# y9c/cutseq

Hardware: AMD Instinct MI355X
Metric: M read-pairs/sec (higher is better)
Workload: dtype u8

## Files before the change

### cutseq_amd/csrc/cutseq_hip.hip

```cpp
#include <hip/hip_runtime.h>

#include <cmath>
#include <cstdarg>
#include <cstdio>
#include <cstdlib>
#include <cstring>
#include <algorithm>
#include <atomic>
#include <map>
#include <new>
#include <string>
#include <thread>
#include <vector>

#include <sys/mman.h>

#include "../../include/cutseq_hip.h"
#include "trim_kernel.hip.inc"
#include "long_kernel.hip.inc"
#include "text_kernels.hip.inc"
#include "deflate_kernels.hip.inc"
#include "info_kernels.hip.inc"

namespace {
// ... 450 lines not shown
  for (int m = 0; m < 2; ++m)
    for (int i = 0; i < cnt[m]; ++i) {
      int rc = build_dev_op(src[m][i], p->host.ops[m][i], i, m + 1);
      if (rc) {
        delete p;
        return rc;
      }
    }
  for (int m = 0; m < 2; ++m) {
    bool seen = false;
    for (int i = 0; i < cnt[m]; ++i) {
      if (seen) p->host.ops[m][i].exists_only = 0;
      seen = seen || p->host.ops[m][i].exists_only != 0;
    }
  }
  bool coded = true;
  for (int m = 0; m < 2; ++m)
    for (int i = 0; i < cnt[m]; ++i) {
      const cs_op &op = p->host.ops[m][i].op;
      if (op.kind != CS_OP_ADAPTER) continue;
      for (int j = 0; j < op.m; ++j) coded = coded && is_acgt(op.seq[j]);
    }
  p->host.coded = coded ? 1 : 0;
  if (coded)
    for (int m = 0; m < 2; ++m)
      for (int i = 0; i < cnt[m]; ++i) {
        csdev::DevOp &d = p->host.ops[m][i];
        if (d.op.kind != CS_OP_ADAPTER) continue;
        for (int j = 0; j < d.op.m; ++j) d.op.seq[j] = (uint8_t)csdev::base_code(d.op.seq[j]);
        d.base_char = csdev::base_code(d.base_char);
      }
  static_assert(csdev::kFnibDwords == 6, "DevOp::fnib");
  for (int m = 0; m < 2; ++m)
    for (int i = 0; i < cnt[m]; ++i) {
      csdev::DevOp &d = p->host.ops[m][i];
      memset(d.eq_tab, 0, sizeof d.eq_tab);
      memset(d.fnib, 0, sizeof d.fnib);
      if (d.op.kind != CS_OP_ADAPTER) continue;
      const int mm = d.op.m;
      for (int ent = 0; ent < 4; ++ent) {
        const int which = (ent == 0) ? 0 : (ent == 1) ? 1 : (ent == 2) ? 3 : 2;
        const uint64_t mask = d.peq[which];
        d.eq_tab[ent * 2] = (uint32_t)mask;
        d.eq_tab[ent * 2 + 1] = (mm >= 1 && mm <= 32) ? ((uint32_t)mask << (32 - mm)) : (uint32_t)(mask >> 32);
      }
      if (coded)
        for (int idx = 0; idx < mm && idx < 32; ++idx)
          d.fnib[idx >> 3] |= (uint32_t)((d.op.seq[d.op.reversed ? mm - 1 - idx : idx] >> 3) & 7u) << (4 * (idx & 7));
    }
  for (int m = 0; m < 2; ++m)
    for (int i = 0; i < cnt[m]; ++i) {
      csdev::DevOp &d = p->host.ops[m][i];
      if (d.op.kind != CS_OP_CUT) continue;
      auto pack = [](const cs_op &o) {
        return (uint32_t)(uint16_t)o.cut_len | ((uint32_t)(o.conditional ? 1u : 0u) << 16) | ((uint32_t)(o.capture & 3u) << 17) |
               ((uint32_t)(o.force_min_len > 0x1fff ? 0x1fffu : o.force_min_len) << 19);
      };
      d.cut_run = 1;
      d.cut_pack[0] = pack(d.op);
    }
  {
    const char *env = getenv("CUTSEQ_CUT_RUNS");
    if (!(env && atoi(env) == 0))
      for (int m = 0; m < 2; ++m)
        for (int i = 0; i < cnt[m];) {
          if (p->host.ops[m][i].op.kind != CS_OP_CUT) {
            ++i;
            continue;
          }
          int j = i;
          while (j < cnt[m] && j - i < csdev::kCutRun && p->host.ops[m][j].op.kind == CS_OP_CUT) {
            p->host.ops[m][i].cut_pack[j - i] = p->host.ops[m][j].cut_pack[0];
            ++j;
          }
          p->host.ops[m][i].cut_run = (uint32_t)(j - i);
          i = j;
        }
  }
  {
    const char *env = getenv("CUTSEQ_PAIR");
    const bool allow = coded && !(env && atoi(env) == 0);
    const char *env_log = getenv("CUTSEQ_LOG_ALWAYS");
    const bool log_always = env_log && atoi(env_log) != 0;
    auto log_friendly = [log_always](int mm, int kk) {
      if (log_always) return true;
      double variants = 0, choose = 1, pw = 1;
      for (int e = 0; e <= kk && e <= mm; ++e) {
        variants += choose * pw;
        choose = choose * (double)(mm - e) / (double)(e + 1);
        pw *= 6.0;
      }
      double space = 1;
      for (int i = 0; i < mm; ++i) space *= 4.0;
      return 300.0 * variants / space < 0.03;
    };
    for (int m = 0; m < 2; ++m) {
      if (allow && cnt[m] >= 1) {
        csdev::DevOp &f = p->host.ops[m][0];
        const bool free_ends = (f.op.align_flags & (CS_QUERY_START | CS_QUERY_STOP)) == (CS_QUERY_START | CS_QUERY_STOP);
        if (f.op.kind == CS_OP_ADAPTER && f.filter_mode == csdev::FILTER_MYERS32 && !f.op.reversed && free_ends &&
            f.op.shortcut == CS_SHORTCUT_NONE && !f.exists_only && log_friendly(f.op.m, f.op.k)) {
          f.solo_first = 1;
          f.quiet_groups = (uint32_t)csdev::quiet_columns((int)f.op.align_flags, f.op.m, f.op.k, nullptr) / 8u;
        }
      }
      if (!allow || cnt[m] < 2) continue;
      csdev::DevOp &a = p->host.ops[m][0];
      const csdev::DevOp &b = p->host.ops[m][1];
      const int ma = a.op.m, ka = a.op.k, mo = a.op.min_overlap;
      const bool ends_free = (b.op.align_flags & (CS_QUERY_START | CS_QUERY_STOP)) == (CS_QUERY_START | CS_QUERY_STOP);
      if (!a.exists_only || a.op.kind != CS_OP_ADAPTER || b.op.kind != CS_OP_ADAPTER || b.exists_only ||
          b.filter_mode != csdev::FILTER_MYERS32 || b.op.reversed || !ends_free || b.op.shortcut != CS_SHORTCUT_NONE ||
          ma + ka > 31 || ka > 14 || !log_friendly(b.op.m, b.op.k))
        continue;
      a.pair_next = 1;
      for (int ent = 0; ent < 4; ++ent) {
        const int which = (ent == 0) ? 0 : (ent == 1) ? 1 : (ent == 2) ? 3 : 2;
        uint32_t fwd = 0;
        for (int i = 0; i < ma; ++i)
          if ((a.peq[which] >> (ma - 1 - i)) & 1ull) fwd |= 1u << i;
        a.eq_fwd[ent] = fwd << (32 - ma);
      }
      for (int j = 1; j <= 32; ++j) {
        int best = -1;
        if (j > ma + ka) best = ka;
        else
          for (int i = mo; i <= ma; ++i) {
            const int d = i > j ? i - j : j - i;
            if (d <= (int)a.op.thr[i] && (int)a.op.thr[i] > best) best = a.op.thr[i];
          }
        a.pair_tn[(j - 1) >> 3] |= (uint32_t)(best + 1) << (4 * ((j - 1) & 7));
      }
      a.quiet_groups = (uint32_t)csdev::quiet_columns((int)b.op.align_flags, b.op.m, b.op.k, a.pair_tn) / 8u;
    }
  }
  *out = p;
  return CS_OK;
}

void cs_plan_destroy(cs_plan *plan) { delete plan; }

int cs_plan_set_max_n(cs_plan *plan, double count) {
  if (!plan) return fail(CS_ERR_ARG, "null plan");
  if (!(count >= 0.0)) return fail(CS_ERR_ARG, "max_n %g: the count must not be negative or NaN", count);
  plan->host.max_n_on = 1;
  plan->host.max_n = count;
  return CS_OK;
}

int cs_plan_set_max_length(cs_plan *plan, uint32_t length) {
  if (!plan) return fail(CS_ERR_ARG, "null plan");
  plan->host.max_length_on = 1;
  plan->host.max_length = length;
  return CS_OK;
}

int cs_plan_set_max_ee(cs_plan *plan, double errors) {
  if (!plan) return fail(CS_ERR_ARG, "null plan");
  if (!(errors >= 0.0)) return fail(CS_ERR_ARG, "max_ee %g: the bound must not be negative or NaN", errors);
  plan->host.max_ee_on = 1;
  plan->host.max_ee = errors;
  for (int b = 0; b < 256; ++b) plan->host.ee_table[b] = pow(10.0, (double)(33 - b) / 10.0);
  return CS_OK;
}

int cs_plan_set_ee_reversed(cs_plan *plan, int reversed) {
  if (!plan) return fail(CS_ERR_ARG, "null plan");
  plan->host.ee_reversed = reversed ? 1u : 0u;
  return CS_OK;
}

int cs_plan_walk_info(const cs_plan *plan, int mate, uint32_t info[6]) {
  if (!plan || !info) return fail(CS_ERR_ARG, "null plan or info");
  if (mate < 1 || mate > 2) return fail(CS_ERR_ARG, "mate %d: 1 or 2", mate);
  memset(info, 0, 6 * sizeof info[0]);
  if (plan->host.n_ops[mate - 1] < 1) return CS_OK;
  const csdev::DevOp &a = plan->host.ops[mate - 1][0];
  info[0] = a.pair_next ? 2u : a.solo_first ? 1u : 0u;
  info[1] = a.quiet_groups;
  for (int i = 0; i < 4; ++i) info[2 + i] = a.pair_tn[i];
  return CS_OK;
}

int cs_plan_set_demux(cs_plan *plan, int mate, int op_index, const uint16_t *table, size_t entries) {
  if (!plan || !table) return fail(CS_ERR_ARG, "null plan or table");
  if (mate < 1 || mate > 2 || op_index < 0 || op_index >= plan->host.n_ops[mate - 1])
    return fail(CS_ERR_ARG, "mate %d op %d: no such op", mate, op_index);
  const cs_op &op = plan->host.ops[mate - 1][op_index].op;
  if (op.kind != CS_OP_DEMUX) return fail(CS_ERR_ARG, "mate %d op %d is not a CS_OP_DEMUX op", mate, op_index);
  if (plan->host.ops[mate - 1][op_index].filter_mode)
    return fail(CS_ERR_ARG, "mate %d op %d: m + k = %d > %d (or CS_DEMUX_BY_OPS) takes cs_plan_set_demux_ops, not a table", mate,
                op_index, op.m + op.k, CS_DEMUX_MAX_PREFIX);
  size_t want = 0, pw = 1;
  for (int l = 0; l <= op.m + op.k; ++l, pw *= 5) want += pw;
  if (entries != want) return fail(CS_ERR_ARG, "demux table: %zu entries, expected %zu for m + k = %d", entries, want, op.m + op.k);
  try {
    plan->demux[mate - 1][op_index].assign(table, table + entries);
  } catch (const std::bad_alloc &) {
    return fail(CS_ERR_NOMEM, "out of memory");
  }
  return CS_OK;
}

namespace {

struct DemuxSegment {
  std::vector<uint8_t> pool;
  std::vector<std::pair<size_t, uint32_t>> first;
};

struct DemuxWalk {
  const std::vector<std::string> &digits;
  int m, k, depth;
  const std::vector<size_t> &block;

  struct Alive {
// ... 1488 lines not shown
```

### cutseq_amd/csrc/trim_kernel.hip.inc

```

#include <type_traits>

namespace csdev {

#ifdef CS_PHASE_TIMERS
struct PhaseTimer {
  uint64_t last;
  uint32_t acc[8];
  uint32_t passes, steps, items;
};
#define CS_T_MARK(T, PHASE)                                   \
  {                                                           \
    const uint64_t cs_now = clock64();                        \
    (T).acc[PHASE] += (uint32_t)(cs_now - (T).last);          \
    (T).last = cs_now;                                        \
  }
#else
#define CS_T_MARK(T, PHASE)
#endif


constexpr int kWave = 64;

constexpr uint32_t kScoreBias = 1024u, kOriginBias = 4096u;
constexpr uint32_t kCostShift = 24, kScoreShift = 13;
constexpr uint32_t kCellZero = (kScoreBias << kScoreShift) | kOriginBias;
constexpr uint32_t kDeltaMatch = 1u << kScoreShift;
constexpr uint32_t kDeltaMismatch = (1u << kCostShift) - (1u << kScoreShift);
constexpr uint32_t kDeltaIndel = (1u << kCostShift) - (2u << kScoreShift);

enum { FILTER_NONE = 0, FILTER_MYERS32 = 1, FILTER_MYERS64 = 2, FILTER_POLY_TAIL = 3, FILTER_POLY_HEAD = 4 };

__host__ __device__ constexpr uint32_t base_code(uint32_t ascii) {
  const uint32_t sel = (ascii >> 1) & 3u;
  const bool ok = ascii == 'A' || ascii == 'C' || ascii == 'G' || ascii == 'T';
  return (sel << 3) | (ok ? 0u : 32u);
}
constexpr int kEqTableBytes = 64;
constexpr int kWaveItemDwords = 4;
constexpr int kCutRun = 4;
constexpr int kQCutoffLow = -1, kQCutoffHigh = 256, kQTermMax = 256;

struct DevFields {
  uint32_t kind, align_flags, reversed, remove, shortcut, match_flag, required, conditional, capture, homopolymer,
      q_base, stat_slot, m, k, min_overlap, force_min_len;
  int32_t cut_len, q_cutoff;
  int32_t length;
};

struct DevOp {
  cs_op op;
  DevFields f;
  uint64_t peq[4];
  uint32_t filter_mode;
  uint32_t base_char;
  uint32_t acgt_only;
  uint32_t thr_mul;
  uint64_t thr_step[2];
  uint32_t eq_tab[kEqTableBytes / 4];
  uint32_t fnib[6];
  uint32_t exists_only;
  uint32_t pair_next;
  uint32_t solo_first;
  uint32_t pair_tn[4];
  uint32_t eq_fwd[4];
  uint32_t cut_run;
  uint32_t cut_pack[kCutRun];
  uint32_t quiet_groups;
};

__host__ __device__ inline int quiet_columns(int flags, int m, int k, const uint32_t *tn) {
  if (flags & CS_REF_START) return 0;
  int q = 0;
  while (q + 8 < m - k && q + 8 <= 32) {
    bool clear = true;
    for (int j = q > 0 ? q : 1; j < q + 8 && tn; ++j)
      clear = clear && ((tn[(j - 1) >> 3] >> (4 * ((j - 1) & 7))) & 15u) == 0u;
    if (!clear) break;
    q += 8;
  }
  return q;
}

struct DevPlan {
  cs_params params;
  int32_t n_ops[2];
  int32_t coded;
  int32_t max_n_on;
  DevOp ops[2][CS_MAX_OPS];
  double max_n;
  uint32_t max_length_on, max_length;
  uint32_t max_ee_on, ee_reversed;
  double max_ee;
  double ee_table[256];
};

constexpr int kMaxPlanSlots = 8;
__constant__ DevPlan c_plans[kMaxPlanSlots];

struct MateArgs {
  const uint32_t *seq;
  const uint8_t *qual;
  const uint16_t *len;
  cs_result *out;
  cs_cap2 *cap2;
  uint8_t *bc;
  uint8_t *xflags;
};

constexpr uint32_t kTileCounters = 8, kTileCounterStride = 32;

struct KArgs {
  MateArgs mate[2];
  unsigned long long *stats;
  uint32_t n_reads;
  uint32_t stride_dw;
  uint32_t lds_stride_dw;
  uint32_t col_dwords;
  uint32_t plan_slot;
  uint32_t *tile_counter;
  uint32_t n_table_ops;
  uint32_t big_tiles;
  uint32_t big_shift, small_shift;
  uint32_t static_units;
  uint4 *defer[2];
  uint32_t batch_knob;
  uint32_t *defer_count;
  uint32_t defer_cap;
  const unsigned long long *gate;
  uint32_t item_slots;
  uint32_t fast_recode;
};

__device__ __forceinline__ uint32_t cell_pack(int cost, int score, int origin) {
  return ((uint32_t)cost << kCostShift) | ((uint32_t)(score + (int)kScoreBias) << kScoreShift) |
         (uint32_t)(origin + (int)kOriginBias);
}
__device__ __forceinline__ int cell_cost(uint32_t c) { return (int)(c >> kCostShift); }
__device__ __forceinline__ int cell_score(uint32_t c) { return (int)((c >> kScoreShift) & 0x7ffu) - (int)kScoreBias; }
__device__ __forceinline__ int cell_origin(uint32_t c) { return (int)(c & 0x1fffu) - (int)kOriginBias; }
constexpr uint32_t kStripScoreBias = 256u, kStripPrioShift = 22;
constexpr uint32_t kStripZero = (kStripScoreBias << kScoreShift) | kOriginBias;
__device__ __forceinline__ uint32_t strip_pack(int cost, int score, int origin) {
  return ((uint32_t)cost << kCostShift) | ((uint32_t)(score + (int)kStripScoreBias) << kScoreShift) |
         (uint32_t)(origin + (int)kOriginBias);
}
__device__ __forceinline__ int strip_score(uint32_t c) {
  return (int)((c >> kScoreShift) & 0x1ffu) - (int)kStripScoreBias;
}

__device__ __forceinline__ int thr_of(const DevOp &d, int L) {
// ... 746 lines not shown
      }
    };
    {
      const uint32_t word = take();
#pragma unroll
      for (int u = 0; u < NB; ++u) q[u] = lookup(word_code<true>(word, DIR > 0 ? u : NB - 1 - u));
      advance();
    }
    __builtin_amdgcn_s_setprio(PRIO_LOOP);
    do {
      const uint32_t word = take();
      advance();
#pragma unroll
      for (int u = 0; u < NB; ++u) {
        myers_step_noscore<false>(st, q[u], 0u);
        q[u] = lookup(word_code<true>(word, DIR > 0 ? u : NB - 1 - u));
        if (u == 3 || u == 7) sample(4);
      }
      j += NB;
    } while (j + NB - 1 <= n);
    __builtin_amdgcn_s_setprio(PRIO_REST);
    int since = 0;
#pragma unroll
    for (int u = 0; u < NB - 1; ++u) {
      if (j <= n) {
        myers_step_noscore<false>(st, q[u], 0u);
        ++j;
        ++since;
        if (since == 4) {
          sample(4);
          since = 0;
        }
      }
    }
    if (since) sample(since);
  } else {
    for (; j <= n; ++j) {
      myers_step_noscore<false>(st, lookup(row_code<true>(row, pos)), 0u);
      pos += DIR;
    }
    if (n > 0) sample(n);
  }
  CS_T_MARK(pt, 1);
  bool none = lowest > 2 * k;
  if (n > 0) {
    const int first_i = RE ? 0 : m;
    const int lo_i = max(first_i, min_overlap);
    const uint32_t pv0 = st.Pv >> sh, mv0 = st.Mv >> sh;
    const int skip = min(max(lo_i - 1, 0), m);
    int cost = 0, thr_i = 0;
    uint32_t pv = pv0, mv = mv0;
    if (skip > 0) {
      const uint32_t below = (skip >= 32) ? ~0u : ((1u << skip) - 1u);
      cost += __popc(pv & below) - __popc(mv & below);
      pv = (skip >= 32) ? 0u : (pv >> skip);
      mv = (skip >= 32) ? 0u : (mv >> skip);
      thr_i = thr_of(d, skip);
    }
    bool any = false;
    for (int i = skip + 1; i <= m; ++i) {
      cost += (int)(pv & 1u) - (int)(mv & 1u);
      pv >>= 1;
      mv >>= 1;
      thr_i += thr_step_bit(d, i);
      any = any || cost <= thr_i;
    }
    none = none && !any;
  }
  return none;
}

__device__ __forceinline__ unsigned long long lds_read_u64(uint32_t addr) { return *(const lds_u64 *)(uintptr_t)addr; }
typedef __attribute__((address_space(3))) uint8_t lds_u8;
__device__ __forceinline__ void lds_write_u8(uint32_t addr, uint32_t imm, uint32_t value) {
  *(lds_u8 *)(uintptr_t)(addr + imm) = (uint8_t)value;
}
__device__ __forceinline__ uint32_t lds_read_u8(uint32_t addr) { return *(const lds_u8 *)(uintptr_t)addr; }
__device__ __forceinline__ uint32_t pk_min_u16(uint32_t a, uint32_t b) {
  uint32_t r;
  asm("v_pk_min_u16 %0, %1, %2" : "=v"(r) : "v"(a), "v"(b));
  return r;
}

struct ItemLog {
  uint32_t slot0;
  uint32_t bytes;
  uint32_t tag_off;
};

template <bool HAS_A>
__device__ __forceinline__ Verdict myers_pair(const DevOp &da, const DevOp &db, int rule, const uint32_t *fnib_b,
                                               const uint32_t *row, int e, bool &a_none, const ItemLog &il CS_T_PARAM) {
  constexpr int NB = 8;
  constexpr int s = 0;
  const int n = e - s;
  const int m = db.f.m, k = db.f.k;
  const bool RS = db.f.align_flags & CS_REF_START;
  const int sh = 32 - m;
  MyersState<uint32_t> st;
  st.Mv = 0;
  st.Pv = RS ? 0u : (m >= 32 ? ~0u : ((1u << m) - 1u));
  const int k1 = k + 1;
  st.score = (RS ? 0 : m) - k1;
  st.Pv = (st.Pv << sh) | ((1u << sh) - 1u);
  const bool exact_by_score = !RS;
  int jfirst = -1, jlast = -1;
  int cmin = 0x7fff, jmin = -1;
  bool tie_next = false;
  uint32_t slot = il.slot0;
  const uint32_t slot_end = il.slot0 + il.bytes;
  bool log_full = false;
  const int ma = da.f.m, ka = da.f.k;
  const int sha = 32 - ma, free_a = ma - (int)da.f.min_overlap;
  MyersState<uint32_t> sa;
  sa.Mv = 0;
  sa.Pv = (((ma >= 32 ? ~0u : ((1u << ma) - 1u)) & ~((1u << free_a) - 1u)) << sha) | ((1u << sha) - 1u);
  sa.score = ma - free_a;
  int flag = 0;
  const uint32_t tn0 = da.pair_tn[0], tn1 = da.pair_tn[1], tn2 = da.pair_tn[2], tn3 = da.pair_tn[3];
  const uint32_t fill_a = (uint32_t)sha, cst4 = (uint32_t)(4 + 2 * ka + 1);
  auto sample_a = [&](uint32_t cst) {
    const int cur = (int)__builtin_popcount(sa.Pv) - (int)(__builtin_popcount(sa.Mv) + fill_a);
    flag |= sa.score + cur - (int)cst;
    sa.score = cur;
  };
  const unsigned long long tn_lo = ((unsigned long long)tn1 << 32) | tn0, tn_hi = ((unsigned long long)tn3 << 32) | tn2;
  auto tn_of = [tn_lo, tn_hi, ka](int j) -> int {
    int t1 = ka + 1;
    if (__ballot(j <= 32)) {
      const unsigned long long w = j <= 16 ? tn_lo : tn_hi;
      const int tj = (int)((uint32_t)(w >> (((uint32_t)(j - 1) & 15u) * 4u)) & 15u);
      t1 = j > 32 ? t1 : tj;
    }
    return t1;
  };
  auto column = [&](uint32_t eb, uint32_t ea, int j) {
    myers_step_la<false>(st, eb, 0u);
    if constexpr (HAS_A) {
      myers_step_la<false>(sa, ea, 0u);
      flag |= sa.score - tn_of(j);
    }
    if (st.score < 0) {
      if (jfirst < 0) jfirst = j;
      jlast = j;
      if (j == jmin + 1 && st.score + k1 == cmin) tie_next = true;
      if (st.score + k1 < cmin) {
        cmin = st.score + k1;
        jmin = j;
        tie_next = false;
      }
    }
  };
  int j = 1;
  if (n >= NB) {
    int wi = 0;
    auto take = [&]() -> uint32_t { return row[wi]; };
    auto advance = [&]() { wi += 1; };
#ifndef CS_PAIR_DEPTH
#define CS_PAIR_DEPTH 2
#endif
    constexpr int QD = CS_PAIR_DEPTH;
    static_assert(NB % QD == 0, "a group's columns must map onto the slots the same way in every group");
    uint32_t qb[QD], qa[QD];
    auto refill = [&](int slot, uint32_t code) {
      const unsigned long long pr = lds_read_u64(code);
      qb[slot] = (uint32_t)pr;
      qa[slot] = (uint32_t)(pr >> 32);
    };
    uint32_t wcur = take();
    advance();
#pragma unroll
    for (int u = 0; u < QD; ++u) refill(u, word_code<true>(wcur, u));
    constexpr int STEADY = 0, EARLY_G = 1, QUIET = 2;
    auto group = [&](auto body_tag, uint32_t tw) {
      constexpr bool EARLY = decltype(body_tag)::value == EARLY_G;
      const uint32_t wnext = take();
      advance();
      if constexpr (decltype(body_tag)::value == QUIET) {
#pragma unroll
        for (int u = 0; u < NB; ++u) {
          myers_step_noscore<false>(st, qb[u % QD], 0u);
          if constexpr (HAS_A) myers_step_noscore<false>(sa, qa[u % QD], 0u);
          refill(u % QD, u + QD < NB ? word_code<true>(wcur, u + QD) : word_code<true>(wnext, u + QD - NB));
        }
        wcur = wnext;
        j += NB;
        return;
      }
      int sc[NB];
#pragma unroll
      for (int u = 0; u < NB; ++u) {
        myers_step_la<false>(st, qb[u % QD], 0u);
        sc[u] = st.score;
        if constexpr (HAS_A && EARLY) {
          myers_step_la<false>(sa, qa[u % QD], 0u);
          flag |= sa.score - (int)((tw >> (4 * u)) & 15u);
        } else if constexpr (HAS_A) {
          myers_step_noscore<false>(sa, qa[u % QD], 0u);
          if (u == 3 || u == 7) sample_a(cst4);
        }
        refill(u % QD, u + QD < NB ? word_code<true>(wcur, u + QD) : word_code<true>(wnext, u + QD - NB));
      }
      wcur = wnext;
      constexpr uint32_t kOr3 = 0xFEu;
      uint32_t any = __builtin_amdgcn_bitop3_b32((uint32_t)sc[0], (uint32_t)sc[1], (uint32_t)sc[2], kOr3);
      any = __builtin_amdgcn_bitop3_b32(any, (uint32_t)sc[3], (uint32_t)sc[4], kOr3);
      any = __builtin_amdgcn_bitop3_b32(any, (uint32_t)sc[5], (uint32_t)sc[6], kOr3);
      any |= (uint32_t)sc[7];
      if ((int)any < 0) {
        if (slot < slot_end) {
#pragma unroll
          for (int u = 0; u < NB; ++u) lds_write_u8(slot, (uint32_t)u, (uint32_t)sc[u]);
          lds_write_u8((slot >> 3) + il.tag_off, 0u, (uint32_t)(j >> 3));
        }
        slot += 8u;
      }
      j += NB;
    };
    __builtin_amdgcn_s_setprio(PRIO_LOOP);
    const int early_groups = (ma + ka + NB - 1) >> 3;
    const int quiet_j = (int)da.quiet_groups * NB + 1;
    if (quiet_j > 1) {
      do group(std::integral_constant<int, QUIET>{}, 0u);
      while (j < quiet_j && j + NB - 1 <= n);
      st.score = (int)__builtin_popcount(st.Pv) - (int)(__builtin_popcount(st.Mv) + (uint32_t)sh) - k1;
      if constexpr (HAS_A) {
        sa.score = (int)__builtin_popcount(sa.Pv) - (int)(__builtin_popcount(sa.Mv) + fill_a);
        const int tq = (int)(da.pair_tn[da.quiet_groups - 1u] >> 28);
        flag |= sa.score - (j == quiet_j ? tq : 0);
      }
    }
    if constexpr (HAS_A) {
      int g = (int)da.quiet_groups;
      while (g < early_groups && j + NB - 1 <= n) {
        group(std::integral_constant<int, EARLY_G>{}, g == 0 ? tn0 : g == 1 ? tn1 : g == 2 ? tn2 : tn3);
        ++g;
      }
    }
    while (j + NB - 1 <= n) group(std::integral_constant<int, STEADY>{}, 0u);
    __builtin_amdgcn_s_setprio(PRIO_REST);
    if (j <= n) {
      int sc[NB];
#pragma unroll
      for (int u = 0; u < NB - 1; ++u) {
        sc[u] = 0x7f;
        if (j + u <= n) {
          uint32_t eb, ea;
          if (u < QD) {
            eb = qb[u];
            ea = qa[u];
          } else {
            const unsigned long long pr = lds_read_u64(word_code<true>(wcur, u));
            eb = (uint32_t)pr;
            ea = (uint32_t)(pr >> 32);
          }
          myers_step_la<false>(st, eb, 0u);
          sc[u] = st.score;
          if constexpr (HAS_A) {
            myers_step_la<false>(sa, ea, 0u);
            flag |= sa.score - tn_of(j + u);
          }
        }
      }
      sc[NB - 1] = 0x7f;
      int any = sc[0];
#pragma unroll
      for (int u = 1; u < NB - 1; ++u) any |= sc[u];
      if (any < 0) {
        if (slot < slot_end) {
#pragma unroll
          for (int u = 0; u < NB; ++u) lds_write_u8(slot, (uint32_t)u, (uint32_t)sc[u]);
          lds_write_u8((slot >> 3) + il.tag_off, 0u, (uint32_t)(j >> 3));
        }
        slot += 8u;
      }
      j = n + 1;
    }
    {
      const uint32_t m80 = 0x80808080u, ones = 0x01010101u;
      const uint32_t stop_at = min(slot, slot_end);
      uint32_t rd = il.slot0;
      while (__ballot(rd < stop_at)) {
        if (rd < stop_at) {
          const unsigned long long sc8 = lds_read_u64(rd);
          const int jg = (int)lds_read_u8((rd >> 3) + il.tag_off) * 8 + 1;
          rd += 8u;
          const uint32_t clo = (uint32_t)sc8 & m80, chi = (uint32_t)(sc8 >> 32) & m80;
          const uint32_t plo = (uint32_t)sc8 ^ m80, phi = (uint32_t)(sc8 >> 32) ^ m80;
          const unsigned long long c64 = ((unsigned long long)chi << 32) | clo;
          if (jfirst < 0) jfirst = jg + (__builtin_ctzll(c64) >> 3);
          jlast = jg + ((63 - __builtin_clzll(c64)) >> 3);
          const uint32_t h00ff = 0x00ff00ffu;
          const uint32_t a0 = plo & h00ff, a1 = (plo >> 8) & h00ff, b0 = phi & h00ff, b1 = (phi >> 8) & h00ff;
          const uint32_t m4 = pk_min_u16(pk_min_u16(a0, a1), pk_min_u16(b0, b1));
          const uint32_t gbyte = min(m4 & 0xffffu, m4 >> 16);
          const int gmin = (int)gbyte - 128 + k1;
          if (jmin == jg - 1 && (int)(plo & 0xffu) - 128 + k1 == cmin) tie_next = true;
          if (gmin < cmin) {
            const uint32_t gb = __builtin_amdgcn_perm(0u, gbyte, 0u);
            const uint32_t xlo = plo ^ gb, xhi = phi ^ gb;
            const uint32_t zlo = (xlo - ones) & ~xlo & m80, zhi = (xhi - ones) & ~xhi & m80;
            const int pos = __builtin_ctzll(((unsigned long long)zhi << 32) | zlo) >> 3;
            cmin = gmin;
            jmin = jg + pos;
            const unsigned long long flipped = ((unsigned long long)phi << 32) | plo;
            tie_next = pos < 7 && (uint32_t)((flipped >> (8 * (pos + 1))) & 0xffull) == gbyte;
          }
        }
      }
      log_full = slot > slot_end;
    }
  } else {
    for (int pos = s; j <= n; ++j, ++pos) {
      const unsigned long long pr = lds_read_u64(row_code<true>(row, pos));
      column((uint32_t)pr, (uint32_t)(pr >> 32), j);
    }
  }
  CS_T_MARK(pt, 1);
  a_none = flag >= 0 && !log_full;
  st.score += k1;
  const int exact_end = (exact_by_score && cmin == 0) ? jmin : -1;
  return myers_verdict<uint32_t, +1, true, true>(db, rule, fnib_b, row, s, e, st, jfirst, jlast, exact_end, cmin, jmin, tie_next);
}

__device__ __forceinline__ uint32_t foreign_flags(const uint32_t *row, int di, uint32_t xrep, int lo, int hi) {
  const uint32_t x = row[di] ^ xrep;
  const uint32_t t = (x | (x >> 1) | (x >> 2)) & 0x11111111u;
  const int first = max(lo - 8 * di, 0), last = min(hi - 8 * di, 8);
  const uint32_t upto = (last >= 8) ? 0xffffffffu : ((1u << (4 * last)) - 1u);
  return t & upto & ~((1u << (4 * first)) - 1u);
}

struct PolyBest {
  bool have;
  int origin, cost, score, len, where;
};

template <bool CODED>
__device__ __forceinline__ Verdict poly_tail(const DevOp &d, int rule, const uint32_t *row, int s, int e) {
  Verdict v = verdict_none(d.f.m);
  const int n = e - s, m = d.f.m, k = d.f.k, min_overlap = d.f.min_overlap;
  const uint32_t X = d.base_char;
  const int lim = min(n, m);
  PolyBest best = {false, 0, 0, 0, 0, 0};
  auto consider = [&](int i, int cost, int score, int origin) {
    if (i >= min_overlap && cost <= thr_of(d, i) &&
        better_candidate(rule, m, best.have, best.origin, best.cost, best.score, best.len, cost, score, origin, i)) {
      best.have = true;
      best.origin = origin;
      best.cost = cost;
      best.score = score;
      best.len = i;
    }
  };
  int b = 0, i_hi = 0;
  if (!CODED) {
    for (int i = 1; i <= lim; ++i) {
      const int nb = b + ((row_code<CODED>(row, e - i) != X) ? 1 : 0);
      if (nb > k) break;
      b = nb;
      i_hi = i;
    }
  } else {
    const uint32_t xrep = (X >> 3) * 0x11111111u;
    const int lo = e - lim;
    for (int di = (e - 1) >> 3; di >= (lo >> 3); --di) {
      const uint32_t f = foreign_flags(row, di, xrep, lo, e);
      const int c = __popc(f);
      const int seg_lo = max(lo, 8 * di);
      if (b + c <= k) {
        b += c;
        i_hi = e - seg_lo;
        continue;
      }
      for (int pos = min(e, 8 * di + 8) - 1; pos >= seg_lo; --pos) {
        const int nb = b + (int)((f >> (4 * (pos - 8 * di))) & 1u);
        if (nb > k) break;
        b = nb;
        i_hi = e - pos;
      }
      break;
    }
  }
  if (i_hi == n && n < m) {
    for (int i = m; i > n; --i) {
      const int cost = (i - n) + b;
      if (cost <= k) consider(i, cost, n - 2 * b, 0);
    }
  }
  if (!CODED) {
    for (int i = i_hi; i >= 1; --i) {
      consider(i, b, i - 2 * b, n - i);
      b -= (row_code<CODED>(row, e - i) != X) ? 1 : 0;
    }
  } else if (i_hi > 0) {
    const uint32_t xrep = (X >> 3) * 0x11111111u;
    const int lo = e - i_hi;
    uint32_t carry = 0;
    for (int di = lo >> 3; di <= ((e - 1) >> 3); ++di) {
      const uint32_t f = foreign_flags(row, di, xrep, lo, e);
      const int c = __popc(f);
      const int seg_lo = max(lo, 8 * di), seg_hi = min(e, 8 * di + 8);
      const int i_left = e - seg_lo;
// ... 678 lines not shown
    if (d == d0) keep &= 0x80808080u << ((s & 3) * 8);
    if (d == d1) keep &= 0x80808080u >> ((3 - ((e - 1) & 3)) * 8);
    const uint32_t x = (row[d] & 0xdfdfdfdfu) ^ 0x4e4e4e4eu;
    n += (uint32_t)__popc(~(((x & 0x7f7f7f7fu) + 0x7f7f7f7fu) | x) & keep);
  }
  return n;
}
__device__ __forceinline__ uint32_t count_n_nibbles(const uint32_t *row, int s, int e) {
  uint32_t n = 0;
  if (e <= s) return 0;
  const int d0 = s >> 3, d1 = (e - 1) >> 3;
  for (int d = d0; d <= d1; ++d) {
    uint32_t keep = 0x11111111u;
    if (d == d0) keep &= 0x11111111u << ((s & 7) * 4);
    if (d == d1) keep &= 0x11111111u >> ((7 - ((e - 1) & 7)) * 4);
    const uint32_t w = row[d];
    n += (uint32_t)__popc(w & (w >> 1) & (w >> 2) & keep);
  }
  return n;
}
__device__ __forceinline__ bool too_many_n(uint32_t n, int len, double count) {
  if (count < 1.0) return len > 0 && (double)n / (double)len > count;
  return (double)n > count;
}
__device__ __forceinline__ double expected_errors(const uint32_t *qrow, int s, int e, const double *table, bool reversed) {
  double ee = 0.0;
  if (e <= s) return ee;
  const int d0 = s >> 2, d1 = (e - 1) >> 2;
  if (!reversed) {
    for (int d = d0; d <= d1; ++d) {
      const uint32_t w = qrow[d];
#pragma unroll
      for (int b = 0; b < 4; ++b) {
        const int p = 4 * d + b;
        if (p >= s && p < e) ee += table[(w >> (8 * b)) & 0xffu];
      }
    }
  } else {
    for (int d = d1; d >= d0; --d) {
      const uint32_t w = qrow[d];
#pragma unroll
      for (int b = 3; b >= 0; --b) {
        const int p = 4 * d + b;
        if (p >= s && p < e) ee += table[(w >> (8 * b)) & 0xffu];
      }
    }
  }
  return ee;
}

enum { MODE_SCAN = 0, MODE_RESOLVE = 1 };

#ifndef CS_SCAN_WAVES
#define CS_SCAN_WAVES 5
#endif
enum { FILT_NONE = 0, FILT_MAXN = 1, FILT_ALL = 2, FILT_ENDS = 3, FILT_NEXTSEQ = 4, FILT_SHORTEN = 5 };
template <bool CODED, bool WIDE, int MODE, int FILT>
__global__ void __launch_bounds__(64, MODE == MODE_RESOLVE ? 4 : CS_SCAN_WAVES) trim_kernel(KArgs a) {
  if (a.gate && *a.gate != ~0ull) return;
  const DevPlan *plan = &c_plans[a.plan_slot];
  extern __shared__ uint32_t smem[];
  constexpr int TILE = kWave;
  constexpr bool SCAN = MODE != MODE_RESOLVE;
  const int tid = threadIdx.x;
  const int mate = blockIdx.y;
  const MateArgs &ma = a.mate[mate];
  const int n_ops = plan->n_ops[mate];
  const uint32_t pw0 = (uint32_t)__builtin_amdgcn_readfirstlane((int)reinterpret_cast<const uint32_t *>(&plan->params)[1]);
  const uint32_t pw1 = (uint32_t)__builtin_amdgcn_readfirstlane((int)reinterpret_cast<const uint32_t *>(&plan->params)[2]);
  static_assert(offsetof(cs_params, min_length) == 4 && offsetof(cs_params, select_rule) == 6 && offsetof(cs_params, use_filter) == 7 &&
                offsetof(cs_params, case_rule) == 8 && offsetof(cs_params, indel_tie) == 9, "cs_params layout");
  const int min_length = (int)(pw0 & 0xffffu);
  const int rule = (int)((pw0 >> 16) & 0xffu);
  const bool use_filter = ((pw0 >> 24) & 0xffu) != 0;
  const bool fold_case = (pw1 & 0xffu) == CS_CASE_FOLD;
  const bool tie_ins = ((pw1 >> 8) & 0xffu) == CS_TIE_INSERTION;
#ifdef CS_PHASE_TIMERS
  const int lane = tid;
#endif

  if (lds_addr_of(smem) != 0u) __builtin_trap();
  __builtin_amdgcn_s_setprio(SCAN ? PRIO_REST : PRIO_RESOLVE);
  uint32_t *cur_tab = smem;
  uint32_t *tile = smem + 20;
  uint32_t *col = tile + (size_t)TILE * a.lds_stride_dw;
  uint32_t *wq = col + a.col_dwords;
  uint32_t *tables = wq + (SCAN ? 0 : kWave * kWaveItemDwords);
  uint32_t *fnibs = tables + a.n_table_ops * (kEqTableBytes / 4);
  uint32_t *sacc = fnibs + a.n_table_ops * kFnibDwords;
  (void)col;
  (void)wq;

  for (int i = tid; i < (int)a.n_table_ops * (kEqTableBytes / 4); i += TILE) {
    const int t = i >> 4;
    tables[i] = t < n_ops ? plan->ops[mate][t].eq_tab[i & 15] : 0u;
  }
  for (int i = tid; i < (int)a.n_table_ops * kFnibDwords; i += TILE) {
    const int t = i / kFnibDwords, w = i - t * kFnibDwords;
    fnibs[i] = (CODED && t < n_ops) ? plan->ops[mate][t].fnib[w] : 0u;
  }
  for (int i = tid; i < kStatWords; i += TILE) sacc[i] = 0;
  if (SCAN && CODED && tid < 4) smem[16 + tid] = (n_ops > 0 && plan->ops[mate][0].pair_next) ? plan->ops[mate][0].eq_fwd[tid] : 0u;

  const uint32_t n_records = SCAN ? 0u : a.defer_count[mate * kTileCounterStride];
  uint32_t batch_rows = TILE;
  if (!SCAN) {
    if (n_records < a.batch_knob * 64u * (uint32_t)gridDim.x) batch_rows = 32;
    if (n_records < a.batch_knob * 32u * (uint32_t)gridDim.x) batch_rows = 16;
  }
  const uint32_t n_refl = SCAN ? 0u : a.defer_count[(4u + (uint32_t)mate) * kTileCounterStride];
  const uint32_t tiles_a = (n_records + batch_rows - 1) / batch_rows;
  const uint32_t n_tiles = SCAN ? (a.n_reads + (uint32_t)TILE - 1) / (uint32_t)TILE : tiles_a + (n_refl + (uint32_t)TILE - 1) / (uint32_t)TILE;
  const uint32_t big_tiles = a.big_tiles, big_units = big_tiles >> a.big_shift;
  const uint32_t big_mask = (1u << a.big_shift) - 1u, small_mask = (1u << a.small_shift) - 1u;
  auto unit_start = [&](uint32_t u) -> uint32_t {
    return (u < big_units) ? (u << a.big_shift) : big_tiles + ((u - big_units) << a.small_shift);
  };
  auto unit_end = [&](uint32_t tile) -> uint32_t {
    return (tile < big_tiles) ? ((tile | big_mask) + 1u) : big_tiles + (((tile - big_tiles) | small_mask) + 1u);
  };
  uint32_t *next_slot = sacc + kStatWords;
  const uint32_t n_counters = min(kTileCounters, (uint32_t)gridDim.x);
  const uint32_t my_counter = blockIdx.x % n_counters;
  uint32_t *counter = a.tile_counter + ((uint32_t)mate * kTileCounters + my_counter) * kTileCounterStride;
  uint32_t *claim = a.defer_count + (2u + (uint32_t)mate) * kTileCounterStride;
  auto next_unit = [&]() -> uint32_t { return a.static_units + my_counter + n_counters * atomicAdd(counter, 1u); };
  if (SCAN) {
    if (tid == 0) *next_slot = unit_start(blockIdx.x < a.static_units ? blockIdx.x : next_unit());
  } else {
    if (tid == 0) *next_slot = atomicAdd(claim, 1u);
  }
  __syncthreads();
  uint32_t tile_id = *next_slot, next_id = 0;
#ifdef CS_PHASE_TIMERS
  PhaseTimer pt;
  pt.last = clock64();
  for (int i = 0; i < 8; ++i) pt.acc[i] = 0;
  pt.passes = pt.steps = pt.items = 0;
#endif

  uint4 *ring = reinterpret_cast<uint4 *>((reinterpret_cast<uintptr_t>(sacc + kStatWords + 4) + 15u) & ~(uintptr_t)15u);
  uint32_t pend_count = 0;
  bool pend_asked = false;
  uint32_t pend_q = 0;
  auto flush_ring = [&]() {
    const uint32_t qb = (uint32_t)__builtin_amdgcn_readfirstlane((int)pend_q);
    const uint32_t lane = wave_lane_fresh();
    if (lane < pend_count) {
      uint4 *rec = a.defer[mate] + (size_t)(qb + lane) * 2u;
      rec[0] = ring[lane * 2];
      rec[1] = ring[lane * 2 + 1];
    }
    pend_count = 0;
    pend_asked = false;
  };
  bool fast_ok = SCAN && CODED && a.fast_recode != 0u, fast_failed = false;
  for (; tile_id < n_tiles; tile_id = next_id) {
  uint32_t lane_fresh = SCAN ? wave_lane_fresh() : threadIdx.x;
  asm volatile("" : "+v"(lane_fresh));
  const int tid = (int)lane_fresh, lane = tid;
  const bool top = !SCAN && tile_id >= tiles_a;
  const uint32_t row0 = top ? (tile_id - tiles_a) * (uint32_t)TILE : tile_id * batch_rows;
  const uint32_t rows_here = top ? min((uint32_t)TILE, n_refl - row0) : min(batch_rows, (SCAN ? a.n_reads : n_records) - row0);
  const bool valid = (uint32_t)tid < rows_here;

  uint32_t gr = row0 + tid;
  int s = 0, e = 0, t0 = 0;
  uint32_t fm = 0, capo = 0, qc = 0;
  uint32_t meta = (uint32_t)CS_DEMUX_NONE << 16;
  uint32_t rec_win = 0, rec_rows = 0, rec_rmax = 0;
  if (!SCAN) {
    uint4 ra = make_uint4(0, 0, 0, 0), rb = make_uint4(0, 0, 0, 0);
    if (valid) {
      const uint4 *rec = a.defer[mate] + (size_t)(top ? a.defer_cap - 1u - gr : gr) * 2u;
      ra = rec[0];
      rb = rec[1];
    }
    gr = ra.x;
    s = (int)(ra.y & 0xffffu);
    e = (int)(ra.y >> 16);
    rec_win = ra.z;
    rec_rows = ra.w;
    t0 = (int)(rb.x >> 24);
    fm = (rb.y & 0xffu) | ((rb.x & 0xffffffu) << 8);
    meta = ((rb.y >> 8) & 0xffu) | ((rb.w >> 24) << 16);
// ... 104 lines not shown
        };
        auto stage = [&](auto fast_tag) -> uint32_t {
          return linear ? stage_coded(fast_tag, std::true_type{}) : stage_coded(fast_tag, std::false_type{});
        };
        bool redo = !fast_ok;
        if (fast_ok) {
          const uint32_t bad = stage(std::true_type{});
          if (a.fast_recode != 2u && __ballot(bad != 0u)) {
            redo = true;
            fast_ok = !fast_failed;
          }
          fast_failed = redo;
        }
        if (redo) (void)stage(std::false_type{});
      } else {
        for (uint32_t dw = tid; dw < total; dw += TILE) {
          const uint32_t r = dw / S;
          tile[r * a.lds_stride_dw + (dw - r * S)] = fold_case ? upper4(src[dw]) : src[dw];
        }
      }
    } else {
      wq[tid] = gr;
      wave_lds_fence();
      const uint32_t total = rows_here * S;
      EncodeConsts ec = encode_consts(fold_case);
      uint32_t r = (uint32_t)tid / S, c = (uint32_t)tid - r * S;
      const uint32_t step_r = (uint32_t)TILE / S, step_c = (uint32_t)TILE - step_r * S;
      constexpr int kBatch = 8;
      for (uint32_t i0 = tid; i0 < total; i0 += (uint32_t)TILE * kBatch) {
        uint32_t w[kBatch], dst[kBatch];
#pragma unroll
        for (int u = 0; u < kBatch; ++u) {
          const uint32_t i = i0 + (uint32_t)u * TILE;
          if (i < total) {
            w[u] = ma.seq[(size_t)wq[r] * S + c];
            dst[u] = CODED ? (tile_b + r * a.lds_stride_dw * 4u + c * 2u) : (r * a.lds_stride_dw + c);
          }
          r += step_r;
          c += step_c;
          if (c >= S) {
            c -= S;
            r += 1;
          }
        }
#pragma unroll
        for (int u = 0; u < kBatch; ++u) {
          const uint32_t i = i0 + (uint32_t)u * TILE;
          if (i < total) {
            if (CODED)
              lds_write_u16(dst[u], 0, encode4_nib_v(w[u], ec));
            else
              tile[dst[u]] = fold_case ? upper4(w[u]) : w[u];
          }
        }
      }
      wave_lds_fence();
    }
  }
  __syncthreads();
  CS_T_MARK(pt, 0);
  const bool same_unit = SCAN && tile_id + 1 < unit_end(tile_id);
  uint32_t fetched = 0;
  if (tid == 0 && !same_unit) fetched = SCAN ? atomic_add_later(counter, 1u) : atomic_add_later(claim, 1u);
  if (SCAN && pend_count >= (uint32_t)kRingRecords / 2) {
    if (tid == 0) pend_q = atomic_add_later(&a.defer_count[mate * kTileCounterStride], pend_count);
    pend_asked = true;
  }
  const uint32_t *wave_rows = tile;
  const uint32_t *myrow = wave_rows + (size_t)lane * a.lds_stride_dw;
  bool deferred = false;
  bool refl = false;
  bool refl_any = false;
  uint32_t refl_q = 0, refl_rank = 0;

  if (SCAN) e = len;
  int t_first = 0;
  if constexpr (SCAN && CODED) {
    const bool pair = use_filter && n_ops >= 2 && plan->ops[mate][0].pair_next;
    const bool solo = use_filter && n_ops >= 1 && plan->ops[mate][0].solo_first;
    if (pair || solo) {
      const int tb = pair ? 1 : 0;
      const DevOp &da = plan->ops[mate][0], &db = plan->ops[mate][tb];
      if (lane < 8) {
        cur_tab[lane * 2] = tables[tb * (kEqTableBytes / 4) + lane * 2 + 1];
        cur_tab[lane * 2 + 1] = (pair && lane < 4) ? smem[16 + lane] : 0u;
      }
      wave_lds_fence();
      bool none = true;
      Verdict vb = verdict_none(db.f.m);
      if (here && len > 0) {
        ItemLog il;
        il.bytes = a.item_slots * 8u;
        il.slot0 = lds_addr_of(ring + kRingRecords * 2) + (uint32_t)lane * il.bytes;
        il.tag_off = (lds_addr_of(ring + kRingRecords * 2) + (uint32_t)TILE * il.bytes) - (lds_addr_of(ring + kRingRecords * 2) >> 3);
        if (pair)
          vb = myers_pair<true>(da, db, rule, fnibs + kFnibDwords, myrow, len, none, il CS_T_ARG);
        else
          vb = myers_pair<false>(da, db, rule, fnibs, myrow, len, none, il CS_T_ARG);
      }
      CS_T_MARK(pt, 2);
      refl = !none;
      const unsigned long long rm = __ballot(refl);
      if (rm) {
        if (lane == 0) refl_q = atomic_add_later(&a.defer_count[(4u + (uint32_t)mate) * kTileCounterStride], (uint32_t)__popcll(rm));
        refl_rank = __builtin_amdgcn_mbcnt_hi((uint32_t)(rm >> 32), __builtin_amdgcn_mbcnt_lo((uint32_t)rm, 0u));
        refl_any = true;
      }
      if (refl) {
        deferred = true;
        rec_win = 0;
        rec_rows = 0xffffffffu;
        rec_rmax = 0xffu;
      } else if (here) {
        if (pair && da.f.required) fm |= CS_F_UNTRIMMED;
#ifdef CS_EXP_REASON
        for (int q = 0; q < 24; ++q) {
          const unsigned long long bm = __ballot(vb.need && vb.reason == q);
          if (bm && lane == 0) atomicAdd(&a.stats[(size_t)mate * kStatWords + ST_OPS + 8 + (q % 12)], (unsigned long long)__popcll(bm) << (q >= 12 ? 32 : 0));
        }
#endif
        if (vb.need) {
          meta += 0x100u;
          deferred = true;
          meta = (meta & 0x00ffffffu) | ((uint32_t)tb << 24);
          rec_win = (uint32_t)vb.j0 | ((uint32_t)vb.j1 << 16) | ((uint32_t)vb.do_end << 31);
          rec_rows = vb.rows;
          rec_rmax = (uint32_t)vb.rmax;
        } else if (vb.found) {
          meta += 1u;
          fm |= (uint32_t)db.f.match_flag | (0x100u << tb);
          if (db.f.remove == CS_REMOVE_BEFORE)
            s = vb.qe;
          else
            e = vb.qs;
        } else if (db.f.required) {
          fm |= CS_F_UNTRIMMED;
        }
      }
      t_first = tb + 1;
    }
  }

  for (int t = t_first; t < n_ops; ++t) {
    const DevOp &d = plan->ops[mate][t];
    const DevFields &op = d.f;
    const bool on = here && !deferred && t >= t0;
    if (!SCAN && !__ballot(on)) continue;
    const int n = e - s;
    const int kind = op.kind;
    if (kind == CS_OP_ADAPTER) {
      const int m = op.m;
      const char *tab = reinterpret_cast<const char *>(tables + t * (kEqTableBytes / 4));
      if (SCAN && (d.filter_mode == FILTER_POLY_TAIL || d.filter_mode == FILTER_POLY_HEAD)) CS_T_MARK(pt, 7);
      Verdict v = verdict_none(m);
      bool poly_lane = false;
      const uint32_t mode = use_filter ? d.filter_mode : (uint32_t)FILTER_NONE;
      if (CODED && mode == FILTER_MYERS32) {
        if (lane < 8) cur_tab[lane * 2] = tables[t * (kEqTableBytes / 4) + lane * 2 + 1];
        wave_lds_fence();
      }
      const bool refilter = !SCAN && on && t == t0 && rec_rmax == 0xffu;
      if (!SCAN && on && t == t0 && !refilter) {
        v.need = 1;
        v.j0 = (int)(rec_win & 0xffffu);
        v.j1 = (int)((rec_win >> 16) & 0x7fffu);
        v.do_end = (int)(rec_win >> 31);
        v.rmax = (int)rec_rmax;
// ... 774 lines not shown
```

### cutseq_amd/switches.py

```python
from __future__ import annotations

import os
from typing import List, NamedTuple, Optional

FLAG_ON, FLAG_OFF, INT, DEVICES, PATH = "flag, default on", "flag, default off", "int", "device list", "path"
PREFIX = "CUTSEQ_"


class Switch(NamedTuple):
    name: str
    kind: str
    default: object
    reader: str
    meaning: str


TABLE = (
    Switch("CUTSEQ_TEXT_PATH", FLAG_ON, True, "python", "0: the record path (host parser and formatter) instead of the text path"),
    Switch("CUTSEQ_GPU_DEFLATE", FLAG_ON, True, "python", "0: gzip outputs are deflated in the host pool, not on the device"),
    Switch("CUTSEQ_GPU_LZ", FLAG_ON, True, "native", "0: the device's gzip members without their LZ77 stage"),
    Switch("CUTSEQ_OWN_INFLATE", FLAG_ON, True, "python", "0: libdeflate inflates gzip input, not the package's decoder"),
    Switch("CUTSEQ_PARALLEL_INFLATE", FLAG_ON, True, "python", "0: single-member gzip input is inflated serially"),
    Switch("CUTSEQ_PAIR", FLAG_ON, True, "native", "0: the chain's leading 5' + 3' ops as two scans, not one merged walk"),
    Switch("CUTSEQ_EXISTS", FLAG_ON, True, "native", "0: the exact filter for the 5' op, not the existence-only scan"),
    Switch("CUTSEQ_CUT_RUNS", FLAG_ON, True, "native", "0: one op-loop turn per CUT op"),
    Switch("CUTSEQ_ITEM_SLOTS", INT, None, "native", "1..16: slots per lane in the leading walk's item log (default: what fits)"),
    Switch("CUTSEQ_FAST_RECODE", INT, 1, "native", "0: exact re-coding of every tile; 2 (tests only): no fallback, mis-codes reads outside ACGTN"),
    Switch("CUTSEQ_PINNED_THP", FLAG_ON, True, "both", "0: page-locked buffers from hipHostMalloc, not from transparent huge pages"),
    Switch("CUTSEQ_DEVICES", DEVICES, None, "python", "GPUs to use, one entry per rank or worker, repeats allowed (default: all)"),
    Switch("CUTSEQ_CHUNK_READS", INT, None, "python", "records per block (default: sized to the input)"),
    Switch("CUTSEQ_HOST_THREADS", INT, None, "native", "bound of the library's host threads; fastq.set_threads writes it (-t/--threads)"),
    Switch("CUTSEQ_HIP_LIB", PATH, None, "python", "the trimming library to load instead of the package's own (A/B builds)"),
    Switch("CUTSEQ_PROGRESS", FLAG_ON, True, "python", "0: no progress line and no Done line"),
    Switch("CUTSEQ_PROFILE", FLAG_OFF, False, "python", "1: seconds per phase, thread and activity on standard error"),
    Switch("CUTSEQ_DISCARD_OUTPUT", FLAG_OFF, False, "python", "1: the writers drop their bytes"),
    Switch("CUTSEQ_DEBUG_INFLATE", FLAG_OFF, False, "python", "1: which chunk of the parallel inflate lost its proof, and how"),
    Switch("CUTSEQ_FAST_EXIT", FLAG_ON, True, "python", "0: the console script unwinds the runtime instead of exiting at once"),
    Switch("CUTSEQ_LOG_ALWAYS", FLAG_OFF, False, "native", "1: every adapter op counts as log-friendly (short adapters through the merged walk)"),
    Switch("CUTSEQ_COL_BYTES", INT, None, "native", "1024..32768: LDS bytes of DP scratch per resolve wave, if more than the plan needs"),
    Switch("CUTSEQ_BATCH_KNOB", INT, 1, "native", "resolve kernel: scales the record counts below which batches shrink to 32 / 16 records"),
    Switch("CUTSEQ_RESOLVE_WAVES", INT, 4, "native", "1..16: resolve waves per CU in pipelined calls"),
    Switch("CUTSEQ_GRID_X", INT, None, "native", "blocks of the scan kernel's grid (default: twice the resident set)"),
    Switch("CUTSEQ_UNITS", INT, None, "native", "three numbers \"big_shift,small_shift,big_pct\": the scan kernel's tile hand-out units"),
)
_BY_KEY = {s.name[len(PREFIX):]: s for s in TABLE}


def _lookup(key: str, *kinds: str) -> Switch:
    s = _BY_KEY[key]
    if s.kind not in kinds or s.reader == "native":
        raise TypeError(f"{s.name} is a {s.kind} switch read by: {s.reader}")
    return s


def enabled(key: str) -> bool:
    s = _lookup(key, FLAG_ON, FLAG_OFF)
    value = os.environ.get(s.name)
    return value != "0" if s.kind == FLAG_ON else value == "1"


def int_value(key: str) -> Optional[int]:
    s = _lookup(key, INT)
    value = os.environ.get(s.name)
    return int(value) if value else s.default


def device_list(key: str, n_default: int) -> List[int]:
    s = _lookup(key, DEVICES)
    value = os.environ.get(s.name)
    return [int(x) for x in value.split(",")] if value else list(range(n_default))


def path(key: str, default: str) -> str:
    s = _lookup(key, PATH)
    return os.environ.get(s.name, default)
```

Measured before the change: 4229.

## Track Myers scores via 8 wildcard rows and chunk table instead of per-column score

```diff
diff --git a/cutseq_amd/csrc/cutseq_hip.hip b/cutseq_amd/csrc/cutseq_hip.hip
--- a/cutseq_amd/csrc/cutseq_hip.hip
+++ b/cutseq_amd/csrc/cutseq_hip.hip
@@ -556,6 +556,8 @@
     const bool allow = coded && !(env && atoi(env) == 0);
     const char *env_log = getenv("CUTSEQ_LOG_ALWAYS");
     const bool log_always = env_log && atoi(env_log) != 0;
+    const char *env_rows = getenv("CUTSEQ_SCORE_ROWS");
+    const bool rows_on = !(env_rows && atoi(env_rows) == 0);
     auto log_friendly = [log_always](int mm, int kk) {
       if (log_always) return true;
       double variants = 0, choose = 1, pw = 1;
@@ -576,6 +578,7 @@
             f.op.shortcut == CS_SHORTCUT_NONE && !f.exists_only && log_friendly(f.op.m, f.op.k)) {
           f.solo_first = 1;
           f.quiet_groups = (uint32_t)csdev::quiet_columns((int)f.op.align_flags, f.op.m, f.op.k, nullptr) / 8u;
+          f.score_rows = (rows_on && f.op.m + 8 <= 32) ? 1u : 0u;
         }
       }
       if (!allow || cnt[m] < 2) continue;
@@ -606,6 +609,7 @@
         a.pair_tn[(j - 1) >> 3] |= (uint32_t)(best + 1) << (4 * ((j - 1) & 7));
       }
       a.quiet_groups = (uint32_t)csdev::quiet_columns((int)b.op.align_flags, b.op.m, b.op.k, a.pair_tn) / 8u;
+      a.score_rows = (rows_on && b.op.m + 8 <= 32) ? 1u : 0u;
     }
   }
   *out = p;
diff --git a/cutseq_amd/csrc/trim_kernel.hip.inc b/cutseq_amd/csrc/trim_kernel.hip.inc
--- a/cutseq_amd/csrc/trim_kernel.hip.inc
+++ b/cutseq_amd/csrc/trim_kernel.hip.inc
@@ -67,6 +67,7 @@
   uint32_t cut_run;
   uint32_t cut_pack[kCutRun];
   uint32_t quiet_groups;
+  uint32_t score_rows;
 };
 
 __host__ __device__ inline int quiet_columns(int flags, int m, int k, const uint32_t *tn) {
@@ -979,6 +980,40 @@
   return r;
 }
 
+constexpr uint32_t kRowsTabAddr = 80u;
+constexpr int kRowsTabDwords = 64;
+typedef __attribute__((address_space(3))) const int8_t lds_ci8;
+__device__ __forceinline__ int lds_read_i8(uint32_t addr) { return *(lds_ci8 *)(uintptr_t)addr; }
+__device__ __forceinline__ uint32_t rows_chunk_entry(uint32_t idx) {
+  const uint32_t p = idx & 15u, mm = idx >> 4;
+  int sum = 0, lowest = 0;
+  for (int i = 0; i < 4; ++i) {
+    lowest = min(lowest, sum);
+    sum += (int)((p >> i) & 1u) - (int)((mm >> i) & 1u);
+  }
+  return (uint32_t)((sum << 4) | (lowest + 3)) & 0xffu;
+}
+__device__ __forceinline__ void rows_item_expand(uint32_t item, uint32_t w) {
+  int run = (int)(int8_t)(w >> 16) + 3;
+#pragma unroll
+  for (int t = 0; t < 8; ++t) {
+    lds_write_u8(item, (uint32_t)(7 - t), (uint32_t)run);
+    run += (int)((w >> t) & 1u) - (int)((w >> (8 + t)) & 1u);
+  }
+}
+__device__ __forceinline__ void myers_step_top(MyersState<uint32_t> &st, uint32_t Eq, uint32_t top) {
+  const uint32_t Pv = st.Pv, Mv = st.Mv;
+  const uint32_t Xv = Eq | Mv;
+  const uint32_t t = (Eq & Pv) + Pv;
+  const uint32_t Xh = __builtin_amdgcn_bitop3_b32(t, Pv, Eq, ((kTtA ^ kTtB) | kTtC) & 0xFFu);
+  const uint32_t Ph = __builtin_amdgcn_bitop3_b32(Mv, Xh, Pv, (kTtA | ~(kTtB | kTtC)) & 0xFFu);
+  const uint32_t Mh = Pv & Xh;
+  st.score += (int)((Ph >> top) & 1u) - (int)((Mh >> top) & 1u);
+  const uint32_t Ph2 = shl1_full_rate(Ph), Mh2 = shl1_full_rate(Mh);
+  st.Pv = __builtin_amdgcn_bitop3_b32(Mh2, Xv, Ph2, (kTtA | ~(kTtB | kTtC)) & 0xFFu);
+  st.Mv = Ph2 & Xv;
+}
+
 struct ItemLog {
   uint32_t slot0;
   uint32_t bytes;
@@ -993,13 +1028,17 @@
   const int n = e - s;
   const int m = db.f.m, k = db.f.k;
   const bool RS = db.f.align_flags & CS_REF_START;
-  const int sh = 32 - m;
+  const bool rows8 = da.score_rows != 0u;
+  const int sh = (rows8 ? 24 : 32) - m;
+  const uint32_t top = rows8 ? 23u : 31u;
+  const int zb = rows8 ? 3 : 0;
   MyersState<uint32_t> st;
   st.Mv = 0;
   st.Pv = RS ? 0u : (m >= 32 ? ~0u : ((1u << m) - 1u));
   const int k1 = k + 1;
   st.score = (RS ? 0 : m) - k1;
   st.Pv = (st.Pv << sh) | ((1u << sh) - 1u);
+  if (rows8) st.Pv |= 0xff000000u;
   const bool exact_by_score = !RS;
   int jfirst = -1, jlast = -1;
   int cmin = 0x7fff, jmin = -1;
@@ -1032,7 +1071,7 @@
     return t1;
   };
   auto column = [&](uint32_t eb, uint32_t ea, int j) {
-    myers_step_la<false>(st, eb, 0u);
+    myers_step_top(st, eb, top);
     if constexpr (HAS_A) {
       myers_step_la<false>(sa, ea, 0u);
       flag |= sa.score - tn_of(j);
@@ -1069,8 +1108,11 @@
 #pragma unroll
     for (int u = 0; u < QD; ++u) refill(u, word_code<true>(wcur, u));
     constexpr int STEADY = 0, EARLY_G = 1, QUIET = 2;
-    auto group = [&](auto body_tag, uint32_t tw) {
+    st.score -= zb;
+    uint32_t cf0 = 0u;
+    auto group = [&](auto body_tag, auto rows_tag, uint32_t tw) {
       constexpr bool EARLY = decltype(body_tag)::value == EARLY_G;
+      constexpr bool ROWS = decltype(rows_tag)::value;
       const uint32_t wnext = take();
       advance();
       if constexpr (decltype(body_tag)::value == QUIET) {
@@ -1081,6 +1123,40 @@
           refill(u % QD, u + QD < NB ? word_code<true>(wcur, u + QD) : word_code<true>(wnext, u + QD - NB));
         }
         wcur = wnext;
+        j += NB;
+        return;
+      }
+      if constexpr (ROWS) {
+#pragma unroll
+        for (int u = 0; u < NB; ++u) {
+          myers_step_noscore<false>(st, qb[u % QD], 0u);
+          if constexpr (HAS_A && EARLY) {
+            myers_step_la<false>(sa, qa[u % QD], 0u);
+            flag |= sa.score - (int)((tw >> (4 * u)) & 15u);
+          } else if constexpr (HAS_A) {
+            myers_step_noscore<false>(sa, qa[u % QD], 0u);
+            if (u == 3 || u == 7) sample_a(cst4);
+          }
+          refill(u % QD, u + QD < NB ? word_code<true>(wcur, u + QD) : word_code<true>(wnext, u + QD - NB));
+        }
+        wcur = wnext;
+        constexpr uint32_t kSel = 0xD8u;
+        const uint32_t hp = st.Pv >> 24, hm = st.Mv >> 24;
+        const uint32_t ilo = __builtin_amdgcn_bitop3_b32(hp, st.Mv >> 20, cf0, kSel);
+        const uint32_t ihi = __builtin_amdgcn_bitop3_b32(st.Pv >> 28, hm, cf0, kSel);
+        const int elo = lds_read_i8(ilo + kRowsTabAddr), ehi = lds_read_i8(ihi + kRowsTabAddr);
+        const int y = st.score - (ehi >> 4);
+        st.score = y - (elo >> 4);
+        const int lo4 = st.score + (int)((uint32_t)elo & 15u), hi4 = y + (int)((uint32_t)ehi & 15u);
+        if ((lo4 | hi4) < 0) {
+          if (slot < slot_end) {
+            lds_write_u8(slot, 0u, hp);
+            lds_write_u8(slot, 1u, hm);
+            lds_write_u8(slot, 2u, (uint32_t)st.score);
+            lds_write_u8((slot >> 3) + il.tag_off, 0u, (uint32_t)(j >> 3));
+          }
+          slot += 8u;
+        }
         j += NB;
         return;
       }
@@ -1118,23 +1194,34 @@
     const int early_groups = (ma + ka + NB - 1) >> 3;
     const int quiet_j = (int)da.quiet_groups * NB + 1;
     if (quiet_j > 1) {
-      do group(std::integral_constant<int, QUIET>{}, 0u);
+      do group(std::integral_constant<int, QUIET>{}, std::false_type{}, 0u);
       while (j < quiet_j && j + NB - 1 <= n);
-      st.score = (int)__builtin_popcount(st.Pv) - (int)(__builtin_popcount(st.Mv) + (uint32_t)sh) - k1;
+      const uint32_t below = rows8 ? 0x00ffffffu : ~0u;
+      st.score = (int)__builtin_popcount(st.Pv & below) - (int)(__builtin_popcount(st.Mv & below) + (uint32_t)sh) - k1 - zb;
       if constexpr (HAS_A) {
         sa.score = (int)__builtin_popcount(sa.Pv) - (int)(__builtin_popcount(sa.Mv) + fill_a);
         const int tq = (int)(da.pair_tn[da.quiet_groups - 1u] >> 28);
         flag |= sa.score - (j == quiet_j ? tq : 0);
       }
     }
-    if constexpr (HAS_A) {
-      int g = (int)da.quiet_groups;
-      while (g < early_groups && j + NB - 1 <= n) {
-        group(std::integral_constant<int, EARLY_G>{}, g == 0 ? tn0 : g == 1 ? tn1 : g == 2 ? tn2 : tn3);
-        ++g;
-      }
-    }
-    while (j + NB - 1 <= n) group(std::integral_constant<int, STEADY>{}, 0u);
+    auto scored_groups = [&](auto rows_tag) {
+      if constexpr (HAS_A) {
+        int g = (int)da.quiet_groups;
+        while (g < early_groups && j + NB - 1 <= n) {
+          group(std::integral_constant<int, EARLY_G>{}, rows_tag, g == 0 ? tn0 : g == 1 ? tn1 : g == 2 ? tn2 : tn3);
+          ++g;
+        }
+      }
+      while (j + NB - 1 <= n) group(std::integral_constant<int, STEADY>{}, rows_tag, 0u);
+    };
+    if (rows8) {
+      cf0 = 0xf0u;
+      asm volatile("" : "+v"(cf0));
+      scored_groups(std::true_type{});
+    } else {
+      scored_groups(std::false_type{});
+    }
+    st.score += zb;
     __builtin_amdgcn_s_setprio(PRIO_REST);
     if (j <= n) {
       int sc[NB];
@@ -1151,7 +1238,7 @@
             eb = (uint32_t)pr;
             ea = (uint32_t)(pr >> 32);
           }
-          myers_step_la<false>(st, eb, 0u);
+          myers_step_top(st, eb, top);
           sc[u] = st.score;
           if constexpr (HAS_A) {
             myers_step_la<false>(sa, ea, 0u);
@@ -1177,6 +1264,14 @@
       const uint32_t m80 = 0x80808080u, ones = 0x01010101u;
       const uint32_t stop_at = min(slot, slot_end);
       uint32_t rd = il.slot0;
+      if (rows8) {
+        const uint32_t tail_tag = (uint32_t)(n >> 3);
+        while (__ballot(rd < stop_at)) {
+          if (rd < stop_at && lds_read_u8((rd >> 3) + il.tag_off) != tail_tag) rows_item_expand(rd, lds_read_u32(rd));
+          rd += 8u;
+        }
+        rd = il.slot0;
+      }
       while (__ballot(rd < stop_at)) {
         if (rd < stop_at) {
           const unsigned long long sc8 = lds_read_u64(rd);
@@ -1216,6 +1311,10 @@
   CS_T_MARK(pt, 1);
   a_none = flag >= 0 && !log_full;
   st.score += k1;
+  if (rows8) {
+    st.Pv <<= 8;
+    st.Mv <<= 8;
+  }
   const int exact_end = (exact_by_score && cmin == 0) ? jmin : -1;
   return myers_verdict<uint32_t, +1, true, true>(db, rule, fnib_b, row, s, e, st, jfirst, jlast, exact_end, cmin, jmin, tie_next);
 }
@@ -2060,7 +2159,8 @@
   if (lds_addr_of(smem) != 0u) __builtin_trap();
   __builtin_amdgcn_s_setprio(SCAN ? PRIO_REST : PRIO_RESOLVE);
   uint32_t *cur_tab = smem;
-  uint32_t *tile = smem + 20;
+  static_assert(kRowsTabAddr == 20 * 4, "the chunk table follows the slack dwords");
+  uint32_t *tile = smem + 20 + (SCAN && CODED ? kRowsTabDwords : 0);
   uint32_t *col = tile + (size_t)TILE * a.lds_stride_dw;
   uint32_t *wq = col + a.col_dwords;
   uint32_t *tables = wq + (SCAN ? 0 : kWave * kWaveItemDwords);
@@ -2079,6 +2179,10 @@
   }
   for (int i = tid; i < kStatWords; i += TILE) sacc[i] = 0;
   if (SCAN && CODED && tid < 4) smem[16 + tid] = (n_ops > 0 && plan->ops[mate][0].pair_next) ? plan->ops[mate][0].eq_fwd[tid] : 0u;
+  if constexpr (SCAN && CODED) {
+    const uint32_t i4 = (uint32_t)tid * 4u;
+    smem[20 + tid] = rows_chunk_entry(i4) | (rows_chunk_entry(i4 + 1u) << 8) | (rows_chunk_entry(i4 + 2u) << 16) | (rows_chunk_entry(i4 + 3u) << 24);
+  }
 
   const uint32_t n_records = SCAN ? 0u : a.defer_count[mate * kTileCounterStride];
   uint32_t batch_rows = TILE;
@@ -2349,7 +2453,8 @@
       const int tb = pair ? 1 : 0;
       const DevOp &da = plan->ops[mate][0], &db = plan->ops[mate][tb];
       if (lane < 8) {
-        cur_tab[lane * 2] = tables[tb * (kEqTableBytes / 4) + lane * 2 + 1];
+        const uint32_t left = tables[tb * (kEqTableBytes / 4) + lane * 2 + 1];
+        cur_tab[lane * 2] = da.score_rows ? (left >> 8) | 0xff000000u : left;
         cur_tab[lane * 2 + 1] = (pair && lane < 4) ? smem[16 + lane] : 0u;
       }
       wave_lds_fence();
diff --git a/cutseq_amd/switches.py b/cutseq_amd/switches.py
--- a/cutseq_amd/switches.py
+++ b/cutseq_amd/switches.py
@@ -25,6 +25,7 @@
     Switch("CUTSEQ_EXISTS", FLAG_ON, True, "native", "0: the exact filter for the 5' op, not the existence-only scan"),
     Switch("CUTSEQ_CUT_RUNS", FLAG_ON, True, "native", "0: one op-loop turn per CUT op"),
     Switch("CUTSEQ_ITEM_SLOTS", INT, None, "native", "1..16: slots per lane in the leading walk's item log (default: what fits)"),
+    Switch("CUTSEQ_SCORE_ROWS", FLAG_ON, True, "native", "0: the leading walk's 3' op keeps a score per column, not the wildcard rows' histories"),
     Switch("CUTSEQ_FAST_RECODE", INT, 1, "native", "0: exact re-coding of every tile; 2 (tests only): no fallback, mis-codes reads outside ACGTN"),
     Switch("CUTSEQ_PINNED_THP", FLAG_ON, True, "both", "0: page-locked buffers from hipHostMalloc, not from transparent huge pages"),
     Switch("CUTSEQ_DEVICES", DEVICES, None, "python", "GPUs to use, one entry per rank or worker, repeats allowed (default: all)"),
```

New measurement: 4267 (median of 6 runs). No clear change (+0.9%).
